# petersn/AtaxxZero

Hardware: AMD Instinct MI355X
Metric: MCTS node-evals/s at 400 sims/move (self-play; games/s beside it) (higher is better)
Workload: dtype bf16

## Files before the change

ataxxzero_amd/csrc/net_kernels.hip:

```cpp
#include <hip/hip_runtime.h>
#include <stdint.h>
#include <math.h>
#include <cmath>
#include <stdlib.h>
#include <stdio.h>
#include <mutex>

#include "azh_host.h"
#include "engine_device.h"

namespace azh {

typedef __attribute__((ext_vector_type(8))) __bf16 bf16x8;
typedef __attribute__((ext_vector_type(4))) __bf16 bf16x4;
typedef __attribute__((ext_vector_type(8))) _Float16 f16x8;
typedef __attribute__((ext_vector_type(4))) _Float16 f16x4;
typedef __attribute__((ext_vector_type(16))) float f32x16;
typedef __attribute__((ext_vector_type(4))) float f32x4;
typedef __attribute__((ext_vector_type(2))) float f32x2;
typedef __attribute__((ext_vector_type(2))) __bf16 bf16x2;
typedef __attribute__((ext_vector_type(2))) _Float16 f16x2;

constexpr int F = 128;
constexpr int OCT = F / 32;
// ... 511 lines not shown
template <> struct Mfma16<AZH_DTYPE_BF16> {
    __device__ static f32x4 mfma(bf16x8 a, bf16x8 b, f32x4 c) { return __builtin_amdgcn_mfma_f32_16x16x32_bf16(a, b, c, 0, 0, 0); }
};
template <> struct Mfma16<AZH_DTYPE_F16> {
    __device__ static f32x4 mfma(f16x8 a, f16x8 b, f32x4 c) { return __builtin_amdgcn_mfma_f32_16x16x32_f16(a, b, c, 0, 0, 0); }
};

struct Geo2 {
    static constexpr int BOARDS = 3;
    static constexpr int NC = 147;
    static constexpr int NT = 10;
    static constexpr int TPW = 5;
    static constexpr int Z = 16;
    static constexpr int NSLOT = 320;
    static constexpr int UB = 16;
    static constexpr int NUNIT = 16;
    static constexpr int CS = NSLOT * UB;
    static constexpr int LDS_BYTES = NUNIT * CS;
    static constexpr int KS_FULL = F / 32, KS_IN = 1;
    __device__ static int real_slot(int img, int c) { return img * (NC + Z) + c; }
    __device__ static int zero_slot(int img, int c) { return NC + ((img * NC + c - NC) & (Z - 1)); }
    __device__ static int ch_off(int slot, int ch) { return (ch >> 3) * CS + slot * UB + ((ch & 7) << 1); }
    __device__ static int vcell_off(int c) { return (c / 40) * CS + 310 * UB + (c % 40) * 4; }
    static constexpr int RING = RING2;
    static constexpr bool SKIP = true;
    __device__ static int tile_cell(int tile, int r);
    static constexpr int NA = 4;
    __device__ static int first_channel(int wave) { return 64 * (wave >> 1); }
    __device__ static int first_a_tile(int wave) { return 4 * (wave >> 1); }
    __device__ static int first_tile(int wave) { return TPW * (wave & 1); }
};

__device__ const unsigned short TILE_CELL[10][16] = {
    {0x010, 0x001, 0x002, 0x003, 0x004, 0x005, 0x006, 0x007, 0x008, 0x009, 0x00a, 0x00b, 0x00c, 0x00d, 0x00e, 0x00f},
    {0x080, 0x081, 0x082, 0x083, 0x084, 0x085, 0x086, 0x087, 0x088, 0x089, 0x08a, 0x08b, 0x08c, 0x08d, 0x08e, 0x07f},
    {0x000, 0x011, 0x012, 0x013, 0x024, 0x025, 0x016, 0x017, 0x018, 0x019, 0x01a, 0x02b, 0x02c, 0x01d, 0x01e, 0x01f},
    {0x020, 0x021, 0x032, 0x033, 0x034, 0x035, 0x026, 0x027, 0x028, 0x039, 0x03a, 0x03b, 0x03c, 0x02d, 0x02e, 0x02f},
    {0x090, 0x091, 0x092, 0x103, 0x104, 0x105, 0x106, 0x107, 0x108, 0x109, 0x10a, 0x10b, 0x10c, 0x10d, 0x10e, 0x10f},
    {0x070, 0x031, 0x062, 0x023, 0x054, 0x015, 0x046, 0x077, 0x038, 0x069, 0x02a, 0x05b, 0x01c, 0x04d, 0x07e, 0x03f},
    {0x030, 0x061, 0x022, 0x053, 0x014, 0x045, 0x076, 0x037, 0x068, 0x029, 0x05a, 0x01b, 0x04c, 0x07d, 0x03e, 0x06f},
    {0x040, 0x041, 0x042, 0x043, 0x044, 0x055, 0x036, 0x047, 0x048, 0x049, 0x04a, 0x04b, 0x05c, 0x03d, 0x04e, 0x04f},
    {0x050, 0x051, 0x052, 0x063, 0x064, 0x065, 0x056, 0x057, 0x058, 0x059, 0x06a, 0x06b, 0x06c, 0x05d, 0x05e, 0x05f},
    {0x060, 0x071, 0x072, 0x073, 0x074, 0x075, 0x066, 0x067, 0x078, 0x079, 0x07a, 0x07b, 0x07c, 0x06d, 0x06e, 0x08f},
};

__device__ inline int Geo2::tile_cell(int tile, int r) { return TILE_CELL[tile][r]; }

#ifndef AZH_RING_THIN
#define AZH_RING_THIN 6
#endif
__device__ const unsigned short TILE_CELL1[4][16] = {
    {0x000, 0x001, 0x002, 0x003, 0x004, 0x005, 0x006, 0x017, 0x018, 0x019, 0x01a, 0x01b, 0x02c, 0x02d, 0x02e, 0x02f},
    {0x030, 0x041, 0x042, 0x043, 0x044, 0x015, 0x016, 0x057, 0x058, 0x059, 0x02a, 0x02b, 0x06c, 0x06d, 0x06e, 0x03f},
    {0x040, 0x081, 0x082, 0x083, 0x054, 0x045, 0x056, 0x107, 0x108, 0x069, 0x05a, 0x06b, 0x10c, 0x10d, 0x07e, 0x06f},
    {0x080, 0x101, 0x102, 0x103, 0x084, 0x055, 0x106, 0x107, 0x108, 0x109, 0x06a, 0x10b, 0x10c, 0x10d, 0x10e, 0x07f},
};
struct Geo2Thin : Geo2 {
    static constexpr int BOARDS = 1;
    static constexpr int NA = 2;
    static constexpr int TPW = 4;
    __device__ static int first_channel(int wave) { return 32 * wave; }
    __device__ static int first_a_tile(int wave) { return 2 * wave; }
    __device__ static int first_tile(int) { return 0; }
    static constexpr int RING = AZH_RING_THIN;
    static constexpr bool SKIP = false;
    __device__ static int tile_cell(int tile, int r) { return TILE_CELL1[tile][r]; }
};
static_assert((3 * Geo2::KS_FULL) % Geo2Thin::RING == 0, "ring phase must be compile-time inside a row");

__device__ inline void cell_xy(int c, int &bl, int &x, int &y)
{
    y = c / 21;
    const int r = c - 21 * y;
    bl = r / 7;
    x = r - 7 * bl;
}

__device__ constexpr bool skip_pair(int chf, int ct, int inner)
{
    return (ct == 0 && inner == 0) || (ct == 1 && inner == 2) || (chf == 0 && ct == 4 && inner == 2);
}

template <int DT> __device__ inline unsigned relu_pack(f32x2 v)
{
    typedef typename Traits<DT>::pair pair;
    const pair p = __builtin_convertvector(v, pair);
    if constexpr (DT == AZH_DTYPE_F16) {
        const pair zero = {0, 0};
        return __builtin_bit_cast(unsigned, __builtin_elementwise_maximum(p, zero));
// ... 310 lines not shown
        for (int i = 0; i < RING2; i++)
#pragma unroll
            for (int t = 0; t < NA; t++)
                tmp[i][t] = a[(i + 2) % RING2][t];
#pragma unroll
        for (int i = 0; i < RING2; i++)
#pragma unroll
            for (int t = 0; t < NA; t++)
                a[i][t] = tmp[i][t];
    }
    if constexpr (STAMP) st[1] = stamp_now();
#pragma unroll
    for (int t = 0; t < NA; t++) {
        const f32x4 t4 = *reinterpret_cast<const f32x4 *>(shift_next + cbase + 16 * t + 4 * kg);
#pragma unroll
        for (int i = 0; i < 4; i++)
            sh[4 * t + i] = t4[i];
    }
    AZH_LAYER_EPILOGUE2
    if constexpr (STAMP) st[2] = stamp_now();
}
#endif

template <int DT, int CHF, bool STAMP, typename G = Geo2>
__device__ inline void tower2_body(const TowerArgs &A, unsigned char *smem, int tile0, int nb, int wave, int lane,
                                   unsigned long long *st, int tbase)
{
    typedef Traits<DT> Tr;
    typedef typename Tr::afrag afrag;
    constexpr int RING2 = G::RING;
    int vmask[G::TPW], cellv[G::TPW];
    {
        const int r = lane & 15;
#pragma unroll
        for (int ct = 0; ct < G::TPW; ct++) {
            const int cv = G::tile_cell(tbase + ct, r);
            cellv[ct] = cv;
            int m = 0;
            if (!(cv & 0x100)) {
                int bl, x, y;
                cell_xy(cv, bl, x, y);
                for (int tap = 0; tap < 9; tap++) {
                    const int xx = x + tap / 3 - 1, yy = y + tap % 3 - 1;
                    if (xx >= 0 && xx < 7 && yy >= 0 && yy < 7)
                        m |= 1 << tap;
                }
            }
            vmask[ct] = m;
#if AZH_OOBZERO
            vmask[ct] = (cv & 0x100) ? 0x3FF : (~m & 0x1FF);
            cellv[ct] = (lane >> 4) * G::CS + (cv & 0xFF) * G::UB;
#endif
        }
    }
    const afrag *wp = reinterpret_cast<const afrag *>(A.conv_w2);
    __amdgpu_buffer_rsrc_t wrsrc = __builtin_amdgcn_make_buffer_rsrc(const_cast<void *>(A.conv_w2), 0, 0x7FFFFFFF, 0x00020000);
#if AZH_FIRST_IM2COL
    const size_t l0 = (size_t)2 * 8 * 64, lf = (size_t)9 * G::KS_FULL * 8 * 64;
#else
    const size_t l0 = (size_t)9 * G::KS_IN * 8 * 64, lf = (size_t)9 * G::KS_FULL * 8 * 64;
#endif
    constexpr int NA = G::NA;
    const int cbase = G::first_channel(wave), atile0 = G::first_a_tile(wave), kg = lane >> 4;
    afrag aring[RING2][G::NA];
#pragma unroll
    for (int i = 0; i < RING2; i++) {
#if AZH_FIRST_IM2COL
        const int step = i;
#else
        const int step = CHF == 0 ? i : 3 * i;
#endif
#pragma unroll
        for (int t = 0; t < NA; t++)
            aring[i][t] = wp[((size_t)step * 8 + atile0 + t) * 64 + lane];
    }
    f32x16 sh;
#pragma unroll
// ... 25 lines not shown
        if constexpr (STAMP) {
            st[12 + 8 * b + 3] = stamp_now();
            if (b < 16)
                st[105 + b] = __builtin_amdgcn_s_memrealtime();
        }
        wp += lf;
    }
}

template <int DT, bool STAMP = false, typename G = Geo2>
__device__ __forceinline__ void tower2_run(const TowerArgs &A, unsigned char *smem, int tile0, int n)
{
    typedef Traits<DT> Tr;
    typedef typename Tr::afrag afrag;
    const int tid = threadIdx.x, lane = tid & 63;
    const int wave = __builtin_amdgcn_readfirstlane(tid >> 6);
    const int nb = (n - tile0) < G::BOARDS ? (n - tile0) : G::BOARDS;
    unsigned long long *st = nullptr;
    if constexpr (STAMP) {
        st = A.stamps + ((size_t)blockIdx.x * OCT + wave) * 128;
        st[0] = stamp_now();
        st[3] = __builtin_amdgcn_s_memrealtime();
    }
    for (int i = tid * 16; i < G::LDS_BYTES; i += NTHREADS * 16)
        *reinterpret_cast<uint4 *>(smem + i) = make_uint4(0, 0, 0, 0);
    __syncthreads();
#if AZH_FIRST_IM2COL
    for (int item = tid; item < G::NC * 5; item += NTHREADS) {
        const int u = item / G::NC, cell = item - u * G::NC;
        int bl, x, y;
        cell_xy(cell, bl, x, y);
        if (bl < nb) {
            int sq0;
            const int game = tower_src(A, tile0 + bl, x, y, sq0);
            const unsigned long long mover = A.boards[2 * (size_t)game + 0];
            const unsigned long long opp = A.boards[2 * (size_t)game + 1];
            const unsigned long long walls = A.masks ? A.masks[game] : A.blockers;
            typename Tr::afrag o;
#pragma unroll
            for (int h = 0; h < 2; h++) {
                const int tap = 2 * u + h;
                const int xx = x + tap / 3 - 1, yy = y + tap % 3 - 1;
                const bool on = tap < 9 && xx >= 0 && xx < 7 && yy >= 0 && yy < 7;
                int sq = 0;
                if (on)
                    (void)tower_src(A, tile0 + bl, xx, yy, sq);
                o[4 * h + 0] = (typename Tr::elem)(on ? 1.0f : 0.0f);
                o[4 * h + 1] = (typename Tr::elem)(float)(on ? (mover >> sq) & 1ULL : 0ULL);
                o[4 * h + 2] = (typename Tr::elem)(float)(on ? (opp >> sq) & 1ULL : 0ULL);
                o[4 * h + 3] = (typename Tr::elem)(float)(on ? (walls >> sq) & 1ULL : 0ULL);
            }
            *reinterpret_cast<typename Tr::afrag *>(smem + u * G::CS + G::real_slot(0, cell) * G::UB) = o;
        }
    }
#else
    for (int cell = tid; cell < G::NC; cell += NTHREADS) {
        int bl, x, y;
        cell_xy(cell, bl, x, y);
        if (bl < nb) {
            int sq;
            const int game = tower_src(A, tile0 + bl, x, y, sq);
            const unsigned long long mover = A.boards[2 * (size_t)game + 0];
            const unsigned long long opp = A.boards[2 * (size_t)game + 1];
            const unsigned long long walls = A.masks ? A.masks[game] : A.blockers;
            typename Tr::quad o;
            o[0] = (typename Tr::elem)1.0f;
            o[1] = (typename Tr::elem)(float)((mover >> sq) & 1ULL);
            o[2] = (typename Tr::elem)(float)((opp >> sq) & 1ULL);
            o[3] = (typename Tr::elem)(float)((walls >> sq) & 1ULL);
            *reinterpret_cast<typename Tr::quad *>(smem + G::ch_off(G::real_slot(0, cell), 0)) = o;
        }
    }
#endif
    __syncthreads();
    if constexpr (G::SKIP) {
        if (wave & 1)
            tower2_body<DT, 1, STAMP, G>(A, smem, tile0, nb, wave, lane, st, G::TPW);
        else
            tower2_body<DT, 0, STAMP, G>(A, smem, tile0, nb, wave, lane, st, 0);
    } else {
        tower2_body<DT, 0, STAMP, G>(A, smem, tile0, nb, wave, lane, st, G::first_tile(wave));
    }
    {
        const afrag *hp = reinterpret_cast<const afrag *>(A.head_w2) + lane;
        const int r = lane & 15, kg = lane >> 4;
        for (int ct = wave; ct < G::NT; ct += OCT) {
            f32x4 acc2[2];
#pragma unroll
            for (int t = 0; t < 2; t++)
#pragma unroll
                for (int i = 0; i < 4; i++)
                    acc2[t][i] = 0.0f;
            const int cell = 16 * ct + r;
            const int slot = cell < G::NC ? G::real_slot(1, cell) : G::zero_slot(1, cell);
#pragma unroll
            for (int ks = 0; ks < G::KS_FULL; ks++) {
                const afrag bfrag = *reinterpret_cast<const afrag *>(smem + (4 * ks + kg) * G::CS + slot * G::UB);
#pragma unroll
                for (int t = 0; t < 2; t++)
                    acc2[t] = Mfma16<DT>::mfma(hp[(size_t)(ks * 2 + t) * 64], bfrag, acc2[t]);
            }
            int bl = 0, x = 0, y = 0;
            if (cell < G::NC)
                cell_xy(cell, bl, x, y);
            if (cell < G::NC && bl < nb) {
                float *dst = A.logits + (size_t)tower_dst(A, tile0 + bl) * 833 + 17 * (7 * x + y);
#pragma unroll
                for (int i = 0; i < 4; i++)
                    dst[4 * kg + i] = acc2[0][i];
                if (kg == 0) {
                    dst[16] = acc2[1][0];
                    *reinterpret_cast<float *>(smem + G::vcell_off(cell)) = acc2[1][1];
                }
            }
        }
    }
    __syncthreads();
    if (tid < nb) {
        const int game = tower_dst(A, tile0 + tid);
        float s = 0.0f;
        for (int c = 0; c < 49; c++)
            s = __builtin_fmaf(*reinterpret_cast<const float *>(smem + G::vcell_off(21 * (c % 7) + 7 * tid + c / 7)), A.fc_w[c], s);
        A.values[game] = tanhf(s + A.fc_b);
    }
    if constexpr (STAMP) {
        st[2] = stamp_now();
        st[104] = __builtin_amdgcn_s_memrealtime();
    }
}

template <int DT, bool STAMP = false>
__global__ __launch_bounds__(NTHREADS, 2) void k_tower2(TowerArgs A, AdvanceHook H)
{
    extern __shared__ __align__(16) unsigned char smem[];
    int wg;
    if (tower_prologue(H, smem, wg))
        return;
    const int n = (A.count ? *A.count : A.n) * (A.sym ? 8 : 1);
    const int tile0 = wg * Geo2::BOARDS;
    if (tile0 >= n)
        return;
    tower2_run<DT, STAMP>(A, smem, tile0, n);
}

template <int DT>
__global__ __launch_bounds__(NTHREADS, 2) void k_tower2_thin(TowerArgs A, AdvanceHook H)
// ... 643 lines not shown
    NetBatch b;
    b.boards = d_b.as<unsigned long long>();
    b.max_n = n;
    b.blockers = blockers;
    b.masks = d_m.as<unsigned long long>();
    b.logits = d_l.as<float>();
    b.values = d_v.as<float>();
    NetOptions o;
    o.thin = mode == AZH_FORWARD_THIN;
    if (mode == AZH_FORWARD_SYM) {
        AZH_HIP(d_tl.alloc((size_t)n * 8 * 833 * 4));
        AZH_HIP(d_tv.alloc((size_t)n * 8 * 4));
        o.sym_logits = d_tl.as<float>();
        o.sym_values = d_tv.as<float>();
    }
    if (int rc = azh_net_launch(net, dtype, b, 0, o))
        return rc;
    AZH_HIP(hipDeviceSynchronize());
    AZH_HIP(hipMemcpy(logits_out, d_l.p, (size_t)n * 833 * 4, hipMemcpyDeviceToHost));
    AZH_HIP(hipMemcpy(values_out, d_v.p, (size_t)n * 4, hipMemcpyDeviceToHost));
    return 0;
}

struct SyntheticBatch {
    DevBuf boards, logits, values;
    NetBatch batch;
    int upload(int n)
    {
        std::vector<unsigned long long> h((size_t)n * 2);
        unsigned long long x = 0x9E3779B97F4A7C15ULL;
        for (int i = 0; i < n; i++) {
            x ^= x << 13; x ^= x >> 7; x ^= x << 17;
            const unsigned long long m = x & 0x1FFFFFFFFFFFFULL;
            x ^= x << 13; x ^= x >> 7; x ^= x << 17;
            h[2 * (size_t)i] = m;
            h[2 * (size_t)i + 1] = x & 0x1FFFFFFFFFFFFULL & ~m;
        }
        AZH_HIP(boards.alloc((size_t)n * 16));
        AZH_HIP(logits.alloc((size_t)n * 833 * 4));
        AZH_HIP(values.alloc((size_t)n * 4));
        AZH_HIP(hipMemcpy(boards.p, h.data(), (size_t)n * 16, hipMemcpyHostToDevice));
        batch.boards = boards.as<unsigned long long>();
        batch.max_n = n;
        batch.logits = logits.as<float>();
        batch.values = values.as<float>();
        return 0;
// ... 64 lines not shown
```

ataxxzero_amd/link.py:

```python
import collections
import ctypes
import os

import numpy as np

from . import build as _build

POLICY_SIZE = 833
FEATURE_SIZE = 196
MAX_MOVES = 256
STAT_COUNT = 16
THIN_MAX_GAMES = 512
DTYPE_F32, DTYPE_BF16, DTYPE_F16 = 0, 1, 2
DTYPES = {"f32": DTYPE_F32, "fp32": DTYPE_F32, "float32": DTYPE_F32, "bf16": DTYPE_BF16,
          "f16": DTYPE_F16, "fp16": DTYPE_F16}
FORWARD_PLAIN, FORWARD_THIN, FORWARD_SYM = 0, 1, 2
LEAF_NONE, LEAF_EVAL, LEAF_TERMINAL, LEAF_ROOT = 0, 1, 2, 3
LEAF_COLLISION = 5
MAX_LEAVES_PER_GAME, MAX_VIRTUAL_LOSS = 64, 16
STAT_COLLISIONS = 15
FLAG_NO_REUSE, FLAG_TIE_FIRST, FLAG_PY_POSTERIOR, FLAG_SAMPLE_POW5, FLAG_KEEP_UNFINISHED, FLAG_TWO_NETS = 1, 2, 4, 8, 16, 32
FLAG_ARENA = 63
FLAG_SYMMETRY_AVG = 128
FLAG_ONE_RANDOM_MOVE = 64
# ... 67 lines not shown

_vp, _i32, _u64, _f32 = ctypes.c_void_p, ctypes.c_int32, ctypes.c_uint64, ctypes.c_float
_P = ctypes.POINTER

SIGNATURES = {
    "azh_last_error": (ctypes.c_char_p, []),
    "azh_device_count": (ctypes.c_int, []),
    "azh_set_device": (ctypes.c_int, [ctypes.c_int]),
    "azh_device_pci_bus_id": (ctypes.c_int, [ctypes.c_int, ctypes.c_char_p, ctypes.c_int]),
    "azh_perft": (ctypes.c_int, [_u64, _u64, _u64, ctypes.c_int, ctypes.c_int, _P(_u64)]),
    "azh_rules_batch": (ctypes.c_int, [ctypes.c_int, _vp, _u64, _vp, _vp, _vp]),
    "azh_makemove_batch": (ctypes.c_int, [ctypes.c_int, _vp, _vp, _vp]),
    "azh_features_batch": (ctypes.c_int, [ctypes.c_int, _vp, _u64, _vp]),
    "azh_random_play": (ctypes.c_int, [ctypes.c_int, _u64, _u64, _u64, _u64, ctypes.c_int, ctypes.c_int,
                                       _vp, _vp, _vp, _vp]),
    "azh_probe_detmath": (ctypes.c_int, [ctypes.c_int, ctypes.c_int, _vp, _vp, _u64, _vp]),
    "azh_alphabeta_search": (ctypes.c_int, [ctypes.c_int, _vp, _u64, _vp, ctypes.c_int, _u64, _vp, _vp, _vp, _vp]),
    "azh_alphabeta_host": (ctypes.c_int, [_u64, _u64, _u64, ctypes.c_int, ctypes.c_int, _u64, _vp, _vp, _vp, _vp]),
    "azh_alphabeta_play": (ctypes.c_int, [ctypes.c_int, _u64, _u64, _u64, _u64, ctypes.c_int, _vp, _vp, ctypes.c_int, _u64,
                                          _vp, ctypes.c_int, ctypes.c_int, _vp, _vp, _vp, _vp, _vp]),
    "azh_net_create": (ctypes.c_int, [ctypes.c_int, ctypes.c_int, _vp, _vp, _f32, _P(_vp)]),
    "azh_net_destroy": (None, [_vp]),
    "azh_net_forward": (ctypes.c_int, [_vp, ctypes.c_int, ctypes.c_int, ctypes.c_int, _vp, _u64, _vp, _vp, _vp]),
    "azh_net_bench": (ctypes.c_int, [_vp, ctypes.c_int, ctypes.c_int, ctypes.c_int, ctypes.c_int, _P(_f32)]),
    "azh_net_tower_choice": (ctypes.c_int, [ctypes.c_int] * 8 + [_vp]),
    "azh_net_stamps": (ctypes.c_int, [_vp, ctypes.c_int, ctypes.c_int, _vp]),
    "azh_engine_create": (ctypes.c_int, [_P(Config), _P(_vp)]),
    "azh_engine_destroy": (None, [_vp]),
    "azh_engine_node_cap": (ctypes.c_int, [_vp]),
    "azh_engine_edge_cap": (ctypes.c_int, [_vp]),
    "azh_engine_select": (ctypes.c_int, [_vp, _P(_i32)]),
    "azh_engine_leaves": (ctypes.c_int, [_vp, _vp, _vp]),
    "azh_engine_leaf_features": (ctypes.c_int, [_vp, _vp, _vp]),
    "azh_engine_eval": (ctypes.c_int, [_vp, _vp, ctypes.c_int]),
    "azh_engine_set_evals": (ctypes.c_int, [_vp, _vp, _vp]),
    "azh_engine_backup": (ctypes.c_int, [_vp]),
    "azh_engine_run": (ctypes.c_int, [_vp, _vp, ctypes.c_int, ctypes.c_int]),
    "azh_engines_run": (ctypes.c_int, [_vp, ctypes.c_int, _vp, ctypes.c_int, ctypes.c_int]),
    "azh_engine_run_arena": (ctypes.c_int, [_vp, _vp, _vp, ctypes.c_int, ctypes.c_int]),
    "azh_engine_sync": (ctypes.c_int, [_vp]),
    "azh_engine_set_visits": (ctypes.c_int, [_vp, ctypes.c_int]),
    "azh_engine_set_thin_batches": (ctypes.c_int, [_vp, ctypes.c_int]),
    "azh_engine_set_leaf_batch": (ctypes.c_int, [_vp, ctypes.c_int, ctypes.c_int]),
    "azh_engine_batch_leaves": (ctypes.c_int, [_vp, _vp, _vp, _vp]),
    "azh_engine_set_batch_evals": (ctypes.c_int, [_vp, _vp, _vp]),
    "azh_engine_set_playout_cap": (ctypes.c_int, [_vp, ctypes.c_int, ctypes.c_int]),
# ... 469 lines not shown
        conv_flat = np.concatenate([np.asarray(a, dtype=np.float32).ravel() for a in conv_weights])
        bn_flat = np.concatenate([np.asarray(a, dtype=np.float32).ravel() for a in bn_params])
        self.blocks, self.filters = blocks, filters
        h = ctypes.c_void_p()
        check(load().azh_net_create(blocks, filters, _ptr(conv_flat), _ptr(bn_flat), bn_eps, ctypes.byref(h)))
        self.h = h

    def _forward(self, mode, leaf_boards, blockers, dtype):
        leaf_boards = np.ascontiguousarray(leaf_boards, dtype=np.uint64).reshape(-1, 2)
        n = len(leaf_boards)
        logits = np.zeros((n, 7, 7, 17), dtype=np.float32)
        values = np.zeros((n, 1), dtype=np.float32)
        masks = None if np.ndim(blockers) == 0 else _board_masks(blockers, n)
        check(load().azh_net_forward(self.h, dtype, mode, n, _ptr(leaf_boards), 0 if masks is not None else int(blockers),
                                     _ptr(masks), _ptr(logits), _ptr(values)))
        return logits, values

    def forward(self, leaf_boards, blockers, dtype=DTYPE_BF16, thin=False):
        return self._forward(FORWARD_THIN if thin else FORWARD_PLAIN, leaf_boards, blockers, dtype)

    def forward_sym(self, leaf_boards, blockers, dtype=DTYPE_BF16):
        return self._forward(FORWARD_SYM, leaf_boards, blockers, dtype)

    def bench(self, n, iters=20, dtype=DTYPE_BF16, thin=False):
        ms = ctypes.c_float(0)
        check(load().azh_net_bench(self.h, dtype, FORWARD_THIN if thin else FORWARD_PLAIN, n, iters, ctypes.byref(ms)))
        return float(ms.value)

    def stamps(self, n, wgs=64):
        out = np.zeros((wgs, 4, 128), dtype=np.uint64)
        check(load().azh_net_stamps(self.h, n, wgs, _ptr(out)))
        return out

    def close(self):
        if getattr(self, "h", None):
            load().azh_net_destroy(self.h)
            self.h = None

    def __del__(self):
        try:
            self.close()
        except Exception:
            pass



# ... 759 lines not shown
```

include/ataxxzero_hip.h:

```cpp
#ifndef ATAXXZERO_HIP_H
#define ATAXXZERO_HIP_H

#include <stdint.h>

#ifdef __cplusplus
extern "C" {
#endif

#define AZH_POLICY_SIZE 833
#define AZH_FEATURE_SIZE 196
#define AZH_MAX_MOVES 256
#define AZH_STAT_COUNT 16

enum { AZH_DTYPE_F32 = 0, AZH_DTYPE_BF16 = 1, AZH_DTYPE_F16 = 2 };
enum { AZH_LEAF_NONE = 0, AZH_LEAF_EVAL = 1, AZH_LEAF_TERMINAL = 2, AZH_LEAF_ROOT = 3, AZH_LEAF_DESCENT = 4,
       AZH_LEAF_COLLISION = 5  };

const char *azh_last_error(void);
int azh_device_count(void);
int azh_set_device(int device);
int azh_device_pci_bus_id(int device, char *buf, int cap);


int azh_perft(uint64_t x, uint64_t o, uint64_t blockers, int turn, int depth, uint64_t *nodes_out);
// ... 15 lines not shown
int azh_alphabeta_search(int n, const uint64_t *boards, uint64_t blockers, const uint64_t *blockers_per_board, int depth,
                         uint64_t node_budget, uint16_t *moves_out, int32_t *values_out, int32_t *depth_done_out,
                         uint64_t *nodes_out);

int azh_alphabeta_host(uint64_t x, uint64_t o, uint64_t blockers, int turn, int depth, uint64_t node_budget,
                       uint16_t *move_out, int32_t *value_out, int32_t *depth_done_out, uint64_t *nodes_out);

int azh_alphabeta_play(int n_games, uint64_t seed, uint64_t x, uint64_t o, uint64_t blockers, int turn,
                       const uint64_t *starts, const uint64_t *blockers_per_game, int depth, uint64_t node_budget,
                       const uint32_t *random_per_2_32, int n_schedule, int max_plies, int32_t *plies, int32_t *results,
                       uint64_t *boards_out, uint16_t *training_moves_out, uint16_t *played_moves_out);

int azh_probe_detmath(int kind, int n, const float *in, const uint32_t *aux, uint64_t seed, uint32_t *out);

typedef struct azh_net azh_net;

int azh_net_create(int blocks, int filters, const float *conv_flat, const float *bn_flat,
                   float bn_eps, azh_net **out);
void azh_net_destroy(azh_net *net);

enum { AZH_FORWARD_PLAIN = 0, AZH_FORWARD_THIN = 1, AZH_FORWARD_SYM = 2 };
int azh_net_forward(azh_net *net, int dtype, int mode, int n, const uint64_t *leaf_boards, uint64_t blockers,
                    const uint64_t *blockers_per_board, float *logits_out, float *values_out);
int azh_net_bench(azh_net *net, int dtype, int mode, int n, int iters, float *ms_out);
typedef struct { char kernel[64]; int32_t boards, threads, lds_bytes, per_cu; } azh_tower_choice;
int azh_net_tower_choice(int filters, int dtype, int thin, int stamped, int pair, int variant1, int six_boards,
                         int lds_range_ok, azh_tower_choice *out);
int azh_net_stamps(azh_net *net, int n, int wgs, uint64_t *out);

typedef struct azh_engine azh_engine;

typedef struct {
    int32_t games;
    int32_t visits;
    int32_t max_plies;
    int32_t edges_per_node;
    float c_puct;
    float dirichlet_alpha;
    float dirichlet_weight;
    int32_t start_turn;
    uint64_t seed;
    uint64_t start_x, start_o, blockers;
    uint32_t flags;
    uint32_t select_budget;
} azh_config;

// ... 244 lines not shown
```

Baseline: 4.509 million.

## Precompute tile tap masks, table-drive first-layer im2col, restage head writeback

Replaces per-lane runtime computation of the tap-validity masks and cell offsets with constant lookup tables, and computes them once before the tower body. Rewrites the first-layer im2col fill to use a packed per-thread item table, zeroing only the pad slots when the tile is full instead of clearing all of LDS. Restructures the head epilogue so logits are copied with vectorized stores from a staged LDS layout and destination indices are cached in LDS, and it preloads value-head operands. Also adds a list-based forward entry point for testing. The hardcoded tables carry a risk of layout mismatches.

```diff
diff --git a/ataxxzero_amd/csrc/net_kernels.hip b/ataxxzero_amd/csrc/net_kernels.hip
--- a/ataxxzero_amd/csrc/net_kernels.hip
+++ b/ataxxzero_amd/csrc/net_kernels.hip
@@ -557,9 +557,12 @@
     __device__ static int zero_slot(int img, int c) { return NC + ((img * NC + c - NC) & (Z - 1)); }
     __device__ static int ch_off(int slot, int ch) { return (ch >> 3) * CS + slot * UB + ((ch & 7) << 1); }
     __device__ static int vcell_off(int c) { return (c / 40) * CS + 310 * UB + (c % 40) * 4; }
+    __device__ static int dst_off(int bl) { return 4 * CS + 310 * UB + bl * 4; }
     static constexpr int RING = RING2;
     static constexpr bool SKIP = true;
     __device__ static int tile_cell(int tile, int r);
+    __device__ static int tile_taps(int tile, int r);
+    __device__ static int tile_off(int tile, int r);
     static constexpr int NA = 4;
     __device__ static int first_channel(int wave) { return 64 * (wave >> 1); }
     __device__ static int first_a_tile(int wave) { return 4 * (wave >> 1); }
@@ -579,7 +582,86 @@
     {0x060, 0x071, 0x072, 0x073, 0x074, 0x075, 0x066, 0x067, 0x078, 0x079, 0x07a, 0x07b, 0x07c, 0x06d, 0x06e, 0x08f},
 };
 
+__device__ const unsigned short TILE_TAPS[10][16] = {
+    {0x049, 0x049, 0x049, 0x049, 0x049, 0x049, 0x1c9, 0x04f, 0x049, 0x049, 0x049, 0x049, 0x049, 0x1c9, 0x04f, 0x049},
+    {0x124, 0x124, 0x124, 0x124, 0x1e4, 0x127, 0x124, 0x124, 0x124, 0x124, 0x124, 0x1e4, 0x127, 0x124, 0x124, 0x124},
+    {0x04f, 0x049, 0x049, 0x049, 0x000, 0x000, 0x000, 0x000, 0x000, 0x000, 0x000, 0x000, 0x000, 0x000, 0x000, 0x000},
+    {0x000, 0x000, 0x000, 0x000, 0x000, 0x000, 0x000, 0x000, 0x000, 0x000, 0x000, 0x000, 0x000, 0x000, 0x000, 0x000},
+    {0x124, 0x124, 0x1e4, 0x3ff, 0x3ff, 0x3ff, 0x3ff, 0x3ff, 0x3ff, 0x3ff, 0x3ff, 0x3ff, 0x3ff, 0x3ff, 0x3ff, 0x3ff},
+    {0x007, 0x007, 0x007, 0x007, 0x007, 0x007, 0x007, 0x007, 0x007, 0x007, 0x007, 0x007, 0x007, 0x007, 0x127, 0x007},
+    {0x1c0, 0x1c0, 0x1c0, 0x1c0, 0x1c9, 0x1c0, 0x1c0, 0x1c0, 0x1c0, 0x1c0, 0x1c0, 0x1c0, 0x1c0, 0x1c0, 0x1c0, 0x1c0},
+    {0x000, 0x000, 0x000, 0x000, 0x000, 0x000, 0x000, 0x000, 0x000, 0x000, 0x000, 0x000, 0x000, 0x000, 0x000, 0x000},
+    {0x000, 0x000, 0x000, 0x000, 0x000, 0x000, 0x000, 0x000, 0x000, 0x000, 0x000, 0x000, 0x000, 0x000, 0x000, 0x000},
+    {0x000, 0x000, 0x000, 0x000, 0x000, 0x000, 0x000, 0x000, 0x000, 0x000, 0x000, 0x000, 0x000, 0x000, 0x000, 0x124},
+};
+__device__ const unsigned short TILE_OFF[10][16] = {
+    {0x100, 0x010, 0x020, 0x030, 0x040, 0x050, 0x060, 0x070, 0x080, 0x090, 0x0a0, 0x0b0, 0x0c0, 0x0d0, 0x0e0, 0x0f0},
+    {0x800, 0x810, 0x820, 0x830, 0x840, 0x850, 0x860, 0x870, 0x880, 0x890, 0x8a0, 0x8b0, 0x8c0, 0x8d0, 0x8e0, 0x7f0},
+    {0x000, 0x110, 0x120, 0x130, 0x240, 0x250, 0x160, 0x170, 0x180, 0x190, 0x1a0, 0x2b0, 0x2c0, 0x1d0, 0x1e0, 0x1f0},
+    {0x200, 0x210, 0x320, 0x330, 0x340, 0x350, 0x260, 0x270, 0x280, 0x390, 0x3a0, 0x3b0, 0x3c0, 0x2d0, 0x2e0, 0x2f0},
+    {0x900, 0x910, 0x920, 0x030, 0x040, 0x050, 0x060, 0x070, 0x080, 0x090, 0x0a0, 0x0b0, 0x0c0, 0x0d0, 0x0e0, 0x0f0},
+    {0x700, 0x310, 0x620, 0x230, 0x540, 0x150, 0x460, 0x770, 0x380, 0x690, 0x2a0, 0x5b0, 0x1c0, 0x4d0, 0x7e0, 0x3f0},
+    {0x300, 0x610, 0x220, 0x530, 0x140, 0x450, 0x760, 0x370, 0x680, 0x290, 0x5a0, 0x1b0, 0x4c0, 0x7d0, 0x3e0, 0x6f0},
+    {0x400, 0x410, 0x420, 0x430, 0x440, 0x550, 0x360, 0x470, 0x480, 0x490, 0x4a0, 0x4b0, 0x5c0, 0x3d0, 0x4e0, 0x4f0},
+    {0x500, 0x510, 0x520, 0x630, 0x640, 0x650, 0x560, 0x570, 0x580, 0x590, 0x6a0, 0x6b0, 0x6c0, 0x5d0, 0x5e0, 0x5f0},
+    {0x600, 0x710, 0x720, 0x730, 0x740, 0x750, 0x660, 0x670, 0x780, 0x790, 0x7a0, 0x7b0, 0x7c0, 0x6d0, 0x6e0, 0x8f0},
+};
+
 __device__ inline int Geo2::tile_cell(int tile, int r) { return TILE_CELL[tile][r]; }
+__device__ inline int Geo2::tile_taps(int tile, int r) { return TILE_TAPS[tile][r]; }
+__device__ inline int Geo2::tile_off(int tile, int r) { return TILE_OFF[tile][r]; }
+
+__device__ const unsigned FEAT_ITEM[245] = {
+    0x00000000, 0x10000010, 0x10400020, 0x10800030, 0x10c00040, 0x11000050, 0x11400060,
+    0x00000150, 0x12200160, 0x12608170, 0x12a10180, 0x12e18190, 0x132201a0, 0x136281b0,
+    0x000002a0, 0x142402b0, 0x146482c0, 0x14a502d0, 0x14e582e0, 0x152602f0, 0x15668300,
+    0x000003f0, 0x16280400, 0x16688410, 0x16a90420, 0x16e98430, 0x172a0440, 0x176a8450,
+    0x00000540, 0x182c0550, 0x186c8560, 0x18ad0570, 0x18ed8580, 0x192e0590, 0x196e85a0,
+    0x00000690, 0x1a3006a0, 0x1a7086b0, 0x1ab106c0, 0x1af186d0, 0x1b3206e0, 0x1b7286f0,
+    0x000007e0, 0x1c3407f0, 0x1c748800, 0x1cb50810, 0x1cf58820, 0x1d360830, 0x1d768840,
+    0x00001400, 0x00241410, 0x00249420, 0x00251430, 0x00259440, 0x00261450, 0x00269460,
+    0x10001550, 0x10681560, 0x10a89570, 0x10e91580, 0x11299590, 0x116a15a0, 0x11aa95b0,
+    0x120016a0, 0x126c16b0, 0x12ac96c0, 0x12ed16d0, 0x132d96e0, 0x136e16f0, 0x13ae9700,
+    0x140017f0, 0x14701800, 0x14b09810, 0x14f11820, 0x15319830, 0x15721840, 0x15b29850,
+    0x16001940, 0x16741950, 0x16b49960, 0x16f51970, 0x17359980, 0x17761990, 0x17b699a0,
+    0x18001a90, 0x18781aa0, 0x18b89ab0, 0x18f91ac0, 0x19399ad0, 0x197a1ae0, 0x19ba9af0,
+    0x1a001be0, 0x1a401bf0, 0x1a801c00, 0x1ac01c10, 0x1b001c20, 0x1b401c30, 0x1b801c40,
+    0x12202800, 0x1260a810, 0x12a12820, 0x12e1a830, 0x13222840, 0x1362a850, 0x13a32860,
+    0x14242950, 0x1464a960, 0x14a52970, 0x14e5a980, 0x15262990, 0x1566a9a0, 0x15a729b0,
+    0x16282aa0, 0x1668aab0, 0x16a92ac0, 0x16e9aad0, 0x172a2ae0, 0x176aaaf0, 0x17ab2b00,
+    0x182c2bf0, 0x186cac00, 0x18ad2c10, 0x18edac20, 0x192e2c30, 0x196eac40, 0x19af2c50,
+    0x1a302d40, 0x1a70ad50, 0x1ab12d60, 0x1af1ad70, 0x1b322d80, 0x1b72ad90, 0x1bb32da0,
+    0x1c342e90, 0x1c74aea0, 0x1cb52eb0, 0x1cf5aec0, 0x1d362ed0, 0x1d76aee0, 0x1db72ef0,
+    0x00382fe0, 0x0038aff0, 0x00393000, 0x0039b010, 0x003a3020, 0x003ab030, 0x003b3040,
+    0x10403c00, 0x10803c10, 0x10c03c20, 0x11003c30, 0x11403c40, 0x11803c50, 0x00003c60,
+    0x1260bd50, 0x12a13d60, 0x12e1bd70, 0x13223d80, 0x1362bd90, 0x13a33da0, 0x00003db0,
+    0x1464bea0, 0x14a53eb0, 0x14e5bec0, 0x15263ed0, 0x1566bee0, 0x15a73ef0, 0x00003f00,
+    0x1668bff0, 0x16a94000, 0x16e9c010, 0x172a4020, 0x176ac030, 0x17ab4040, 0x00004050,
+    0x186cc140, 0x18ad4150, 0x18edc160, 0x192e4170, 0x196ec180, 0x19af4190, 0x000041a0,
+    0x1a70c290, 0x1ab142a0, 0x1af1c2b0, 0x1b3242c0, 0x1b72c2d0, 0x1bb342e0, 0x000042f0,
+    0x1c74c3e0, 0x1cb543f0, 0x1cf5c400, 0x1d364410, 0x1d76c420, 0x1db74430, 0x00004440,
+    0x0024d000, 0x00255010, 0x0025d020, 0x00265030, 0x0026d040, 0x00275050, 0x00005060,
+    0x0028d150, 0x00295160, 0x0029d170, 0x002a5180, 0x002ad190, 0x002b51a0, 0x000051b0,
+    0x002cd2a0, 0x002d52b0, 0x002dd2c0, 0x002e52d0, 0x002ed2e0, 0x002f52f0, 0x00005300,
+    0x0030d3f0, 0x00315400, 0x0031d410, 0x00325420, 0x0032d430, 0x00335440, 0x00005450,
+    0x0034d540, 0x00355550, 0x0035d560, 0x00365570, 0x0036d580, 0x00375590, 0x000055a0,
+    0x0038d690, 0x003956a0, 0x0039d6b0, 0x003a56c0, 0x003ad6d0, 0x003b56e0, 0x000056f0,
+    0x000057e0, 0x000057f0, 0x00005800, 0x00005810, 0x00005820, 0x00005830, 0x00005840,
+};
+
+constexpr int STAGE_SPLIT = 32 * 17;
+__device__ const unsigned short HEAD_STAGE[160] = {
+    0x0000, 0x01dc, 0x03b8, 0x0594, 0x0770, 0x14cc, 0x16a8, 0x2800, 0x29dc, 0x2bb8, 0x2d94, 0x2f70, 0x3ccc, 0x3ea8, 0x5000, 0x51dc,
+    0x53b8, 0x5594, 0x5770, 0x64cc, 0x66a8, 0x0044, 0x0220, 0x03fc, 0x05d8, 0x07b4, 0x1510, 0x16ec, 0x2844, 0x2a20, 0x2bfc, 0x2dd8,
+    0x2fb4, 0x3d10, 0x3eec, 0x5044, 0x5220, 0x53fc, 0x55d8, 0x57b4, 0x6510, 0x66ec, 0x0088, 0x0264, 0x0440, 0x061c, 0x07f8, 0x1554,
+    0x1730, 0x2888, 0x2a64, 0x2c40, 0x2e1c, 0x2ff8, 0x3d54, 0x3f30, 0x5088, 0x5264, 0x5440, 0x561c, 0x57f8, 0x6554, 0x6730, 0x00cc,
+    0x02a8, 0x0484, 0x0660, 0x083c, 0x1598, 0x1774, 0x28cc, 0x2aa8, 0x2c84, 0x2e60, 0x303c, 0x3d98, 0x3f74, 0x50cc, 0x52a8, 0x5484,
+    0x5660, 0x583c, 0x6598, 0x6774, 0x0110, 0x02ec, 0x04c8, 0x06a4, 0x1400, 0x15dc, 0x17b8, 0x2910, 0x2aec, 0x2cc8, 0x2ea4, 0x3c00,
+    0x3ddc, 0x3fb8, 0x5110, 0x52ec, 0x54c8, 0x56a4, 0x6400, 0x65dc, 0x67b8, 0x0154, 0x0330, 0x050c, 0x06e8, 0x1444, 0x1620, 0x17fc,
+    0x2954, 0x2b30, 0x2d0c, 0x2ee8, 0x3c44, 0x3e20, 0x3ffc, 0x5154, 0x5330, 0x550c, 0x56e8, 0x6444, 0x6620, 0x67fc, 0x0198, 0x0374,
+    0x0550, 0x072c, 0x1488, 0x1664, 0x1840, 0x2998, 0x2b74, 0x2d50, 0x2f2c, 0x3c88, 0x3e64, 0x4040, 0x5198, 0x5374, 0x5550, 0x572c,
+    0x6488, 0x6664, 0x6840, 0xffff, 0xffff, 0xffff, 0xffff, 0xffff, 0xffff, 0xffff, 0xffff, 0xffff, 0xffff, 0xffff, 0xffff, 0xffff,
+};
 
 #ifndef AZH_RING_THIN
 #define AZH_RING_THIN 6
@@ -589,6 +671,18 @@
     {0x030, 0x041, 0x042, 0x043, 0x044, 0x015, 0x016, 0x057, 0x058, 0x059, 0x02a, 0x02b, 0x06c, 0x06d, 0x06e, 0x03f},
     {0x040, 0x081, 0x082, 0x083, 0x054, 0x045, 0x056, 0x107, 0x108, 0x069, 0x05a, 0x06b, 0x10c, 0x10d, 0x07e, 0x06f},
     {0x080, 0x101, 0x102, 0x103, 0x084, 0x055, 0x106, 0x107, 0x108, 0x109, 0x06a, 0x10b, 0x10c, 0x10d, 0x10e, 0x07f},
+};
+__device__ const unsigned short TILE_TAPS1[4][16] = {
+    {0x04f, 0x049, 0x049, 0x049, 0x049, 0x049, 0x1c9, 0x000, 0x000, 0x000, 0x000, 0x1c0, 0x000, 0x000, 0x000, 0x000},
+    {0x1c0, 0x000, 0x000, 0x000, 0x000, 0x007, 0x000, 0x000, 0x000, 0x000, 0x007, 0x000, 0x000, 0x000, 0x000, 0x007},
+    {0x000, 0x124, 0x124, 0x124, 0x007, 0x1c0, 0x000, 0x3ff, 0x3ff, 0x007, 0x1c0, 0x000, 0x3ff, 0x3ff, 0x127, 0x1c0},
+    {0x124, 0x3ff, 0x3ff, 0x3ff, 0x1e4, 0x000, 0x3ff, 0x3ff, 0x3ff, 0x3ff, 0x000, 0x3ff, 0x3ff, 0x3ff, 0x3ff, 0x124},
+};
+__device__ const unsigned short TILE_OFF1[4][16] = {
+    {0x000, 0x010, 0x020, 0x030, 0x040, 0x050, 0x060, 0x170, 0x180, 0x190, 0x1a0, 0x1b0, 0x2c0, 0x2d0, 0x2e0, 0x2f0},
+    {0x300, 0x410, 0x420, 0x430, 0x440, 0x150, 0x160, 0x570, 0x580, 0x590, 0x2a0, 0x2b0, 0x6c0, 0x6d0, 0x6e0, 0x3f0},
+    {0x400, 0x810, 0x820, 0x830, 0x540, 0x450, 0x560, 0x070, 0x080, 0x690, 0x5a0, 0x6b0, 0x0c0, 0x0d0, 0x7e0, 0x6f0},
+    {0x800, 0x010, 0x020, 0x030, 0x840, 0x550, 0x060, 0x070, 0x080, 0x090, 0x6a0, 0x0b0, 0x0c0, 0x0d0, 0x0e0, 0x7f0},
 };
 struct Geo2Thin : Geo2 {
     static constexpr int BOARDS = 1;
@@ -600,6 +694,8 @@
     static constexpr int RING = AZH_RING_THIN;
     static constexpr bool SKIP = false;
     __device__ static int tile_cell(int tile, int r) { return TILE_CELL1[tile][r]; }
+    __device__ static int tile_taps(int tile, int r) { return TILE_TAPS1[tile][r]; }
+    __device__ static int tile_off(int tile, int r) { return TILE_OFF1[tile][r]; }
 };
 static_assert((3 * Geo2::KS_FULL) % Geo2Thin::RING == 0, "ring phase must be compile-time inside a row");
 
@@ -956,37 +1052,28 @@
 }
 #endif
 
+template <typename G> __device__ inline void tower2_lane_tiles(int tbase, int lane, int (&vmask)[G::TPW], int (&cellv)[G::TPW])
+{
+    const int r = lane & 15;
+#pragma unroll
+    for (int ct = 0; ct < G::TPW; ct++) {
+#if AZH_OOBZERO
+        vmask[ct] = G::tile_taps(tbase + ct, r);
+        cellv[ct] = (lane >> 4) * G::CS + G::tile_off(tbase + ct, r);
+#else
+        vmask[ct] = ~G::tile_taps(tbase + ct, r) & 0x1FF;
+        cellv[ct] = G::tile_cell(tbase + ct, r);
+#endif
+    }
+}
+
 template <int DT, int CHF, bool STAMP, typename G = Geo2>
 __device__ inline void tower2_body(const TowerArgs &A, unsigned char *smem, int tile0, int nb, int wave, int lane,
-                                   unsigned long long *st, int tbase)
+                                   unsigned long long *st, const int (&vmask)[G::TPW], const int (&cellv)[G::TPW])
 {
     typedef Traits<DT> Tr;
     typedef typename Tr::afrag afrag;
     constexpr int RING2 = G::RING;
-    int vmask[G::TPW], cellv[G::TPW];
-    {
-        const int r = lane & 15;
-#pragma unroll
-        for (int ct = 0; ct < G::TPW; ct++) {
-            const int cv = G::tile_cell(tbase + ct, r);
-            cellv[ct] = cv;
-            int m = 0;
-            if (!(cv & 0x100)) {
-                int bl, x, y;
-                cell_xy(cv, bl, x, y);
-                for (int tap = 0; tap < 9; tap++) {
-                    const int xx = x + tap / 3 - 1, yy = y + tap % 3 - 1;
-                    if (xx >= 0 && xx < 7 && yy >= 0 && yy < 7)
-                        m |= 1 << tap;
-                }
-            }
-            vmask[ct] = m;
-#if AZH_OOBZERO
-            vmask[ct] = (cv & 0x100) ? 0x3FF : (~m & 0x1FF);
-            cellv[ct] = (lane >> 4) * G::CS + (cv & 0xFF) * G::UB;
-#endif
-        }
-    }
     const afrag *wp = reinterpret_cast<const afrag *>(A.conv_w2);
     __amdgpu_buffer_rsrc_t wrsrc = __builtin_amdgcn_make_buffer_rsrc(const_cast<void *>(A.conv_w2), 0, 0x7FFFFFFF, 0x00020000);
 #if AZH_FIRST_IM2COL
@@ -1058,38 +1145,53 @@
         st[0] = stamp_now();
         st[3] = __builtin_amdgcn_s_memrealtime();
     }
+    int vmask[G::TPW], cellv[G::TPW];
+    tower2_lane_tiles<G>(G::first_tile(wave), lane, vmask, cellv);
+#if AZH_FIRST_IM2COL
+    static_assert(NTHREADS == G::NUNIT * G::Z && G::NSLOT - (2 * G::NC + G::Z) <= G::Z && NTHREADS >= G::NC, "one store per slot");
+    if (nb < G::BOARDS) {
+        for (int i = tid * 16; i < G::LDS_BYTES; i += NTHREADS * 16)
+            *reinterpret_cast<uint4 *>(smem + i) = make_uint4(0, 0, 0, 0);
+        __syncthreads();
+    } else {
+        const int u = tid >> 4, j = tid & 15;
+        if (tid < G::NC) {
+#pragma unroll
+            for (int pad = 5; pad < 8; pad++)
+                *reinterpret_cast<uint4 *>(smem + pad * G::CS + tid * G::UB) = make_uint4(0, 0, 0, 0);
+        }
+        *reinterpret_cast<uint4 *>(smem + u * G::CS + (G::NC + j) * G::UB) = make_uint4(0, 0, 0, 0);
+        if (j < G::NSLOT - (2 * G::NC + G::Z))
+            *reinterpret_cast<uint4 *>(smem + u * G::CS + (2 * G::NC + G::Z + j) * G::UB) = make_uint4(0, 0, 0, 0);
+    }
+    static_assert(NTHREADS >= 5 * 49, "one item per thread and board");
+    constexpr unsigned ONE = DT == AZH_DTYPE_BF16 ? 0x3F80u : 0x3C00u;
+    const unsigned item = FEAT_ITEM[tid < 5 * 49 ? tid : 0];
+#pragma unroll
+    for (int bl = 0; bl < G::BOARDS; bl++) {
+        if (bl < nb && tid < 5 * 49) {
+            int sq0;
+            const int game = tower_src(A, tile0 + bl, 0, 0, sq0);
+            const unsigned long long mover = A.boards[2 * (size_t)game + 0];
+            const unsigned long long opp = A.boards[2 * (size_t)game + 1];
+            const unsigned long long walls = A.masks ? A.masks[game] : A.blockers;
+            unsigned q[4];
+#pragma unroll
+            for (int h = 0; h < 2; h++) {
+                const unsigned f = item >> (15 + 7 * h);
+                const unsigned on = (f >> 6) & 1u;
+                int sq;
+                (void)tower_src(A, tile0 + bl, (int)(f & 7u), (int)((f >> 3) & 7u), sq);
+                q[2 * h + 0] = (on | (((unsigned)(mover >> sq) & on) << 16)) * ONE;
+                q[2 * h + 1] = (((unsigned)(opp >> sq) & on) | (((unsigned)(walls >> sq) & on) << 16)) * ONE;
+            }
+            *reinterpret_cast<uint4 *>(smem + (item & 0x7FFFu) + bl * (7 * G::UB)) = make_uint4(q[0], q[1], q[2], q[3]);
+        }
+    }
+#else
     for (int i = tid * 16; i < G::LDS_BYTES; i += NTHREADS * 16)
         *reinterpret_cast<uint4 *>(smem + i) = make_uint4(0, 0, 0, 0);
     __syncthreads();
-#if AZH_FIRST_IM2COL
-    for (int item = tid; item < G::NC * 5; item += NTHREADS) {
-        const int u = item / G::NC, cell = item - u * G::NC;
-        int bl, x, y;
-        cell_xy(cell, bl, x, y);
-        if (bl < nb) {
-            int sq0;
-            const int game = tower_src(A, tile0 + bl, x, y, sq0);
-            const unsigned long long mover = A.boards[2 * (size_t)game + 0];
-            const unsigned long long opp = A.boards[2 * (size_t)game + 1];
-            const unsigned long long walls = A.masks ? A.masks[game] : A.blockers;
-            typename Tr::afrag o;
-#pragma unroll
-            for (int h = 0; h < 2; h++) {
-                const int tap = 2 * u + h;
-                const int xx = x + tap / 3 - 1, yy = y + tap % 3 - 1;
-                const bool on = tap < 9 && xx >= 0 && xx < 7 && yy >= 0 && yy < 7;
-                int sq = 0;
-                if (on)
-                    (void)tower_src(A, tile0 + bl, xx, yy, sq);
-                o[4 * h + 0] = (typename Tr::elem)(on ? 1.0f : 0.0f);
-                o[4 * h + 1] = (typename Tr::elem)(float)(on ? (mover >> sq) & 1ULL : 0ULL);
-                o[4 * h + 2] = (typename Tr::elem)(float)(on ? (opp >> sq) & 1ULL : 0ULL);
-                o[4 * h + 3] = (typename Tr::elem)(float)(on ? (walls >> sq) & 1ULL : 0ULL);
-            }
-            *reinterpret_cast<typename Tr::afrag *>(smem + u * G::CS + G::real_slot(0, cell) * G::UB) = o;
-        }
-    }
-#else
     for (int cell = tid; cell < G::NC; cell += NTHREADS) {
         int bl, x, y;
         cell_xy(cell, bl, x, y);
@@ -1109,17 +1211,21 @@
     }
 #endif
     __syncthreads();
+    if (tid < nb)
+        *reinterpret_cast<int *>(smem + G::dst_off(tid)) = tower_dst(A, tile0 + tid);
     if constexpr (G::SKIP) {
         if (wave & 1)
-            tower2_body<DT, 1, STAMP, G>(A, smem, tile0, nb, wave, lane, st, G::TPW);
+            tower2_body<DT, 1, STAMP, G>(A, smem, tile0, nb, wave, lane, st, vmask, cellv);
         else
-            tower2_body<DT, 0, STAMP, G>(A, smem, tile0, nb, wave, lane, st, 0);
+            tower2_body<DT, 0, STAMP, G>(A, smem, tile0, nb, wave, lane, st, vmask, cellv);
     } else {
-        tower2_body<DT, 0, STAMP, G>(A, smem, tile0, nb, wave, lane, st, G::first_tile(wave));
-    }
+        tower2_body<DT, 0, STAMP, G>(A, smem, tile0, nb, wave, lane, st, vmask, cellv);
+    }
+    const int lane_end = (int)__builtin_amdgcn_mbcnt_hi(~0u, __builtin_amdgcn_mbcnt_lo(~0u, 0u));
+    const int tid_end = wave * 64 + lane_end;
     {
-        const afrag *hp = reinterpret_cast<const afrag *>(A.head_w2) + lane;
-        const int r = lane & 15, kg = lane >> 4;
+        const afrag *hp = reinterpret_cast<const afrag *>(A.head_w2) + lane_end;
+        const int r = lane_end & 15, kg = lane_end >> 4;
         for (int ct = wave; ct < G::NT; ct += OCT) {
             f32x4 acc2[2];
 #pragma unroll
@@ -1131,33 +1237,50 @@
             const int slot = cell < G::NC ? G::real_slot(1, cell) : G::zero_slot(1, cell);
 #pragma unroll
             for (int ks = 0; ks < G::KS_FULL; ks++) {
-                const afrag bfrag = *reinterpret_cast<const afrag *>(smem + (4 * ks + kg) * G::CS + slot * G::UB);
+                const afrag bfrag = *reinterpret_cast<const afrag *>(smem + ((4 * ks + kg) * G::NSLOT + slot) * G::UB);
 #pragma unroll
                 for (int t = 0; t < 2; t++)
                     acc2[t] = Mfma16<DT>::mfma(hp[(size_t)(ks * 2 + t) * 64], bfrag, acc2[t]);
             }
-            int bl = 0, x = 0, y = 0;
-            if (cell < G::NC)
-                cell_xy(cell, bl, x, y);
-            if (cell < G::NC && bl < nb) {
-                float *dst = A.logits + (size_t)tower_dst(A, tile0 + bl) * 833 + 17 * (7 * x + y);
+            const int stage = HEAD_STAGE[cell];
+            if (stage < nb * (2 * G::CS)) {
 #pragma unroll
                 for (int i = 0; i < 4; i++)
-                    dst[4 * kg + i] = acc2[0][i];
+                    *reinterpret_cast<float *>(smem + stage + 4 * (4 * kg + i)) = acc2[0][i];
                 if (kg == 0) {
-                    dst[16] = acc2[1][0];
+                    *reinterpret_cast<float *>(smem + stage + 4 * 16) = acc2[1][0];
                     *reinterpret_cast<float *>(smem + G::vcell_off(cell)) = acc2[1][1];
                 }
             }
         }
     }
     __syncthreads();
-    if (tid < nb) {
-        const int game = tower_dst(A, tile0 + tid);
+    const bool values = wave == OCT - 1 && lane_end < nb;
+    float vc[49], fw[49];
+    if (values) {
+#pragma unroll
+        for (int c = 0; c < 49; c++) {
+            vc[c] = *reinterpret_cast<const float *>(smem + G::vcell_off(21 * (c % 7) + 7 * lane_end + c / 7));
+            fw[c] = A.fc_w[c];
+        }
+    }
+    typedef float f32x4u __attribute__((ext_vector_type(4), aligned(4)));
+    static_assert(STAGE_SPLIT % 4 == 0 && NTHREADS > 833 / 4, "a piece lies in one unit; a piece per thread");
+    for (int bl = 0; bl < nb; bl++) {
+        float *row = A.logits + (size_t)*reinterpret_cast<const int *>(smem + G::dst_off(bl)) * 833;
+        const int f = 4 * tid_end;
+        const unsigned char *src = smem + (f < STAGE_SPLIT ? 2 * bl * G::CS + 4 * f : (2 * bl + 1) * G::CS + 4 * (f - STAGE_SPLIT));
+        if (f + 4 <= 833)
+            *reinterpret_cast<f32x4u *>(row + f) = *reinterpret_cast<const f32x4 *>(src);
+        else if (f < 833)
+            row[f] = *reinterpret_cast<const float *>(src);
+    }
+    if (values) {
         float s = 0.0f;
+#pragma unroll
         for (int c = 0; c < 49; c++)
-            s = __builtin_fmaf(*reinterpret_cast<const float *>(smem + G::vcell_off(21 * (c % 7) + 7 * tid + c / 7)), A.fc_w[c], s);
-        A.values[game] = tanhf(s + A.fc_b);
+            s = __builtin_fmaf(vc[c], fw[c], s);
+        A.values[*reinterpret_cast<const int *>(smem + G::dst_off(lane_end))] = tanhf(s + A.fc_b);
     }
     if constexpr (STAMP) {
         st[2] = stamp_now();
@@ -1847,6 +1970,73 @@
     return 0;
 }
 
+extern "C" int azh_net_forward_lists(azh_net *net_a, azh_net *net_b, int dtype, int mode, int games, const uint64_t *boards,
+                                     uint64_t blockers, const uint64_t *masks, const int32_t *list_a, int na,
+                                     const int32_t *list_b, int nb, float *logits_inout, float *values_inout)
+{
+    if (!net_a || games <= 0 || !boards || !list_a || na <= 0 || !logits_inout || !values_inout || (net_b && (!list_b || nb <= 0)))
+        return azh_fail(-1, "azh_net_forward_lists: bad argument");
+    if (mode != AZH_FORWARD_PLAIN && mode != AZH_FORWARD_THIN && mode != AZH_FORWARD_SYM)
+        return azh_fail(-2, "azh_net_forward_lists: bad mode %d", mode);
+    if (net_b && mode == AZH_FORWARD_SYM)
+        return azh_fail(-2, "azh_net_forward_lists: two nets in one launch are not averaged over symmetries");
+    if (masks && blockers)
+        return azh_fail(-2, "azh_net_forward_lists: a mask per board AND blockers: the wall plane has one source");
+    const int total = na + (net_b ? nb : 0);
+    std::vector<int> h_list(list_a, list_a + na);
+    if (net_b)
+        h_list.insert(h_list.end(), list_b, list_b + nb);
+    for (int g : h_list)
+        if (g < 0 || g >= games)
+            return azh_fail(-2, "azh_net_forward_lists: list entry %d outside the %d boards", g, games);
+    const int h_count[2] = {na, nb};
+    DevBuf d_b, d_m, d_l, d_v, d_tl, d_tv, d_list, d_count;
+    AZH_HIP(d_b.alloc((size_t)games * 16));
+    AZH_HIP(d_l.alloc((size_t)games * 833 * 4));
+    AZH_HIP(d_v.alloc((size_t)games * 4));
+    AZH_HIP(d_list.alloc((size_t)total * 4));
+    AZH_HIP(d_count.alloc(sizeof h_count));
+    AZH_HIP(hipMemcpy(d_b.p, boards, (size_t)games * 16, hipMemcpyHostToDevice));
+    AZH_HIP(hipMemcpy(d_l.p, logits_inout, (size_t)games * 833 * 4, hipMemcpyHostToDevice));
+    AZH_HIP(hipMemcpy(d_v.p, values_inout, (size_t)games * 4, hipMemcpyHostToDevice));
+    AZH_HIP(hipMemcpy(d_list.p, h_list.data(), (size_t)total * 4, hipMemcpyHostToDevice));
+    AZH_HIP(hipMemcpy(d_count.p, h_count, sizeof h_count, hipMemcpyHostToDevice));
+    if (masks) {
+        AZH_HIP(d_m.alloc((size_t)games * 8));
+        AZH_HIP(hipMemcpy(d_m.p, masks, (size_t)games * 8, hipMemcpyHostToDevice));
+    }
+    NetBatch b;
+    b.boards = d_b.as<unsigned long long>();
+    b.list = d_list.as<int>();
+    b.count = d_count.as<int>();
+    b.max_n = total;
+    b.blockers = blockers;
+    b.masks = d_m.as<unsigned long long>();
+    b.logits = d_l.as<float>();
+    b.values = d_v.as<float>();
+    NetOptions o;
+    o.thin = mode == AZH_FORWARD_THIN;
+    if (mode == AZH_FORWARD_SYM) {
+        AZH_HIP(d_tl.alloc((size_t)na * 8 * 833 * 4));
+        AZH_HIP(d_tv.alloc((size_t)na * 8 * 4));
+        o.sym_logits = d_tl.as<float>();
+        o.sym_values = d_tv.as<float>();
+    }
+    if (net_b) {
+        const int rc = azh_net_launch_pair(net_a, net_b, dtype, b, d_list.as<int>() + na, d_count.as<int>() + 1, 0, o);
+        if (rc == 1)
+            return azh_fail(-2, "azh_net_forward_lists: no two-net launch for these nets in this process");
+        if (rc)
+            return rc;
+    } else if (int rc = azh_net_launch(net_a, dtype, b, 0, o)) {
+        return rc;
+    }
+    AZH_HIP(hipDeviceSynchronize());
+    AZH_HIP(hipMemcpy(logits_inout, d_l.p, (size_t)games * 833 * 4, hipMemcpyDeviceToHost));
+    AZH_HIP(hipMemcpy(values_inout, d_v.p, (size_t)games * 4, hipMemcpyDeviceToHost));
+    return 0;
+}
+
 struct SyntheticBatch {
     DevBuf boards, logits, values;
     NetBatch batch;
diff --git a/ataxxzero_amd/link.py b/ataxxzero_amd/link.py
--- a/ataxxzero_amd/link.py
+++ b/ataxxzero_amd/link.py
@@ -113,6 +113,8 @@
     "azh_net_create": (ctypes.c_int, [ctypes.c_int, ctypes.c_int, _vp, _vp, _f32, _P(_vp)]),
     "azh_net_destroy": (None, [_vp]),
     "azh_net_forward": (ctypes.c_int, [_vp, ctypes.c_int, ctypes.c_int, ctypes.c_int, _vp, _u64, _vp, _vp, _vp]),
+    "azh_net_forward_lists": (ctypes.c_int, [_vp, _vp, ctypes.c_int, ctypes.c_int, ctypes.c_int, _vp, _u64, _vp, _vp, ctypes.c_int,
+                                             _vp, ctypes.c_int, _vp, _vp]),
     "azh_net_bench": (ctypes.c_int, [_vp, ctypes.c_int, ctypes.c_int, ctypes.c_int, ctypes.c_int, _P(_f32)]),
     "azh_net_tower_choice": (ctypes.c_int, [ctypes.c_int] * 8 + [_vp]),
     "azh_net_stamps": (ctypes.c_int, [_vp, ctypes.c_int, ctypes.c_int, _vp]),
@@ -628,6 +630,20 @@
     def forward_sym(self, leaf_boards, blockers, dtype=DTYPE_BF16):
         return self._forward(FORWARD_SYM, leaf_boards, blockers, dtype)
 
+    def forward_lists(self, leaf_boards, blockers, leaf_list, dtype=DTYPE_BF16, mode=FORWARD_PLAIN, other=None, other_list=None,
+                      fill=0.0):
+        leaf_boards = np.ascontiguousarray(leaf_boards, dtype=np.uint64).reshape(-1, 2)
+        n = len(leaf_boards)
+        logits = np.full((n, 7, 7, 17), fill, dtype=np.float32)
+        values = np.full((n, 1), fill, dtype=np.float32)
+        masks = None if np.ndim(blockers) == 0 else _board_masks(blockers, n)
+        la = np.ascontiguousarray(leaf_list, dtype=np.int32).ravel()
+        lb = None if other is None else np.ascontiguousarray(other_list, dtype=np.int32).ravel()
+        check(load().azh_net_forward_lists(self.h, other.h if other is not None else None, dtype, mode, n, _ptr(leaf_boards),
+                                           0 if masks is not None else int(blockers), _ptr(masks), _ptr(la), len(la),
+                                           _ptr(lb), 0 if lb is None else len(lb), _ptr(logits), _ptr(values)))
+        return logits, values
+
     def bench(self, n, iters=20, dtype=DTYPE_BF16, thin=False):
         ms = ctypes.c_float(0)
         check(load().azh_net_bench(self.h, dtype, FORWARD_THIN if thin else FORWARD_PLAIN, n, iters, ctypes.byref(ms)))
diff --git a/include/ataxxzero_hip.h b/include/ataxxzero_hip.h
--- a/include/ataxxzero_hip.h
+++ b/include/ataxxzero_hip.h
@@ -61,6 +61,9 @@
 enum { AZH_FORWARD_PLAIN = 0, AZH_FORWARD_THIN = 1, AZH_FORWARD_SYM = 2 };
 int azh_net_forward(azh_net *net, int dtype, int mode, int n, const uint64_t *leaf_boards, uint64_t blockers,
                     const uint64_t *blockers_per_board, float *logits_out, float *values_out);
+int azh_net_forward_lists(azh_net *net_a, azh_net *net_b, int dtype, int mode, int games, const uint64_t *boards,
+                          uint64_t blockers, const uint64_t *masks, const int32_t *list_a, int na, const int32_t *list_b, int nb,
+                          float *logits_inout, float *values_inout);
 int azh_net_bench(azh_net *net, int dtype, int mode, int n, int iters, float *ms_out);
 typedef struct { char kernel[64]; int32_t boards, threads, lds_bytes, per_cu; } azh_tower_choice;
 int azh_net_tower_choice(int filters, int dtype, int thin, int stamped, int pair, int variant1, int six_boards,
```

Measured after the change: 4.532 million (median of 6 runs). Within noise of the previous version (+0.5%).
